# williamleif/GraphSAGE

Hardware: NVIDIA H100
Metric: seed_nodes_per_sec (higher is better)
Workload: dtype f32

## Files before the change

### graphsage_b200/_lib.py

```python
import ctypes
import os

import torch

_HERE = os.path.dirname(os.path.abspath(__file__))
LIB_PATH = os.path.join(_HERE, "csrc", "libgraphsage_b200.so")

ABI_VERSION = 2
GS_F32, GS_BF16, GS_F64, GS_I8ROW = 0, 1, 2, 3
ACT_NONE, ACT_RELU = 0, 1
COMBINE_ADD, COMBINE_CONCAT = 0, 1
MATH_FP32_SIMT, MATH_TF32X3, MATH_TF32, MATH_BF16 = 0, 1, 2, 3
CSR_MEAN, CSR_MEAN_SELF, CSR_MAX, CSR_SUM = 0, 1, 2, 3
MAX_SEGMENTS = 4

c_i32, c_i64, c_u64, c_vp = ctypes.c_int32, ctypes.c_int64, ctypes.c_uint64, ctypes.c_void_p


class Segment(ctypes.Structure):
    _fields_ = [("self_ids", c_vp), ("neigh_ids", c_vp), ("self_row0", c_i64), ("neigh_row0", c_i64),
                ("n", c_i64), ("k", c_i32), ("_pad", c_i32), ("out_row0", c_i64)]


MAX_SHARDS = 16


class ShardedTable(ctypes.Structure):
    _fields_ = [("base", c_vp * MAX_SHARDS), ("row_start", c_i64 * (MAX_SHARDS + 1)), ("n_shards", c_i32),
                ("my_shard", c_i32), ("n_global_rows", c_i64), ("zero_row", c_i64), ("remap", c_vp)]


class GemmPart(ctypes.Structure):
    _fields_ = [("A", c_vp), ("lda", c_i64), ("K", c_i32), ("B", c_vp), ("ldb", c_i64), ("N", c_i32)]


class RowRange(ctypes.Structure):
    _fields_ = [("ids", c_vp), ("row0", c_i64), ("n", c_i64)]


class GemmRowIds(ctypes.Structure):
    _fields_ = [("n_table_rows", c_i64), ("n_ranges", c_i32), ("_pad", c_i32), ("ranges", RowRange * MAX_SEGMENTS)]


MAX_EMBED_LISTS = 8
# ... 1 lines not shown
UNIQUE_DRAW_BUDGET = 1 << 20
WALK_MAX_WALKS = 1 << 20
WALK_MAX_LEN = 33
WALK_PQ_MIN, WALK_PQ_MAX = 1e-4, 1e4
MAX_BLOCK_LAYERS = 8
MAX_FANOUT = 256


class EmbedGradList(ctypes.Structure):
    _fields_ = [("ids", c_vp), ("grad", c_vp), ("ldg", c_i64), ("n", c_i64), ("group", c_i32), ("scale", ctypes.c_float)]


class DropoutSite(ctypes.Structure):
    _fields_ = [("seed", c_u64), ("call", ctypes.c_uint32), ("rate", ctypes.c_float), ("call_dev", c_vp)]


_SIGNATURES = {
    "gs_version": (c_i32, []),
    "gs_last_error_string": (ctypes.c_char_p, []),
    "gs_set_tuning": (c_i32, [ctypes.c_char_p, c_i32]),
    "gs_sample_padded": (c_i32, [c_vp, c_i64, c_i32, c_vp, c_i64, c_i32, c_vp, c_u64, c_u64, c_vp, c_vp, c_vp]),
    "gs_sample_padded_khop": (c_i32, [c_vp, c_i64, c_i32, c_vp, c_i64, ctypes.POINTER(c_i32), c_i32, c_u64, c_u64, c_vp,
                                      ctypes.POINTER(c_vp), c_vp]),
    "gs_build_padded_adj": (c_i32, [c_vp, c_vp, c_i64, c_i32, c_vp, c_u64, c_u64, c_vp, c_vp, c_vp]),
    "gs_sample_unigram": (c_i32, [c_vp, c_i64, c_i32, c_u64, c_u64, c_vp, c_vp, c_vp]),
    "gs_sample_unigram_unique": (c_i32, [c_vp, c_i64, c_i32, c_u64, c_u64, c_vp, c_vp, c_vp, c_vp]),
    "gs_sample_csr": (c_i32, [c_vp, c_vp, c_i64, c_vp, c_i64, c_i32, c_i32, c_u64, c_u64, c_vp, c_i32, c_vp, c_vp]),
    "gs_perm_prefix_host": (c_i32, [c_u64, c_u64, c_i32, c_i32, ctypes.POINTER(c_i32)]),
    "gs_gather_rows": (c_i32, [c_vp, c_i32, c_i64, c_i32, c_i64, c_vp, c_i64, c_vp, c_i64, c_vp]),
    "gs_gather_mean": (c_i32, [c_vp, c_i32, c_i64, c_i32, c_i64, ctypes.POINTER(Segment), c_i32, c_i32, c_vp, c_vp,
                               c_i64, c_vp]),
    "gs_gather_mean_sharded": (c_i32, [ctypes.POINTER(ShardedTable), c_i32, c_i32, c_i64, ctypes.POINTER(Segment), c_i32,
                                       c_i32, c_i32, c_vp, c_vp, c_vp, c_i64, c_vp]),
    "gs_halo_begin": (c_i32, [c_vp, c_i64, c_vp, c_vp]),
    "gs_halo_claim": (c_i32, [ctypes.POINTER(ShardedTable), c_vp, c_i64, c_vp, c_vp, c_vp, c_i64, c_vp]),
    "gs_halo_fetch": (c_i32, [ctypes.POINTER(ShardedTable), c_i32, c_i64, c_vp, c_vp, c_i64, c_vp, c_i64, c_vp]),
    "gs_halo_translate": (c_i32, [ctypes.POINTER(ShardedTable), c_vp, c_i64, c_vp, c_vp, c_vp]),
    "gs_translate_ids": (c_i32, [ctypes.POINTER(ShardedTable), c_vp, c_i64, c_vp, c_vp]),
    "gs_gather_rows_sharded": (c_i32, [ctypes.POINTER(ShardedTable), c_i32, c_i32, c_i64, c_vp, c_i64, c_vp, c_i64, c_vp]),
    "gs_shard_alloc": (c_i32, [c_i64, ctypes.POINTER(c_vp)]),
    "gs_shard_free": (c_i32, [c_vp]),
    "gs_ipc_export": (c_i32, [c_vp, ctypes.c_char_p]),
    "gs_ipc_import": (c_i32, [ctypes.c_char_p, ctypes.POINTER(c_vp)]),
    "gs_ipc_close": (c_i32, [c_vp]),
    "gs_host_register": (c_i32, [c_vp, c_i64, ctypes.POINTER(c_vp)]),
    "gs_host_unregister": (c_i32, [c_vp]),
# ... 157 lines not shown
```

### graphsage_b200/csrc/gather.cu

```cuda
#include "common.cuh"

namespace gs {

struct SegTable {
  gs_segment s[GS_MAX_SEGMENTS];
  int32_t n_segments;
  int64_t total_rows;
};

__device__ __forceinline__ int find_segment(const SegTable& t, int64_t r, int64_t& local) {
  int si = 0;
  int64_t base = 0, end = 0;
#pragma unroll
  for (int q = 0; q < GS_MAX_SEGMENTS - 1; ++q) {
    if (q < t.n_segments - 1) {
      end += t.s[q].n;
      if (r >= end) {
        base = end;
        si = q + 1;
      }
    }
  }
  local = r - base;
  return si;
// ... 223 lines not shown
  if (threadIdx.x == 0) {
    mbar_init(&bar[0], 1);
    mbar_init(&bar[1], 1);
    fence_mbar_init();
  }
  if constexpr (kDrop) {
    if (threadIdx.x < 2 * GS_MAX_SEGMENTS) {
      const int s = threadIdx.x % GS_MAX_SEGMENTS;
      drop_off[threadIdx.x] = drop_call_offset(threadIdx.x < GS_MAX_SEGMENTS ? drop.neigh[s] : drop.self[s]);
    }
  }
  __syncthreads();
  const int ncol4 = (int)(out_pitch >> 2);
  const int row_f4 = row_bytes >> 4;
  const size_t buf_bytes = (size_t)kGroupRows * row_bytes;
  const int self_rows = (include_self || out_self) ? 1 : 0;

  int64_t r_issue = blockIdx.x;
  int g_issue = 0;
  auto issue = [&](int buf) -> bool {
    if (r_issue >= tab.total_rows) return false;
    int64_t i;
    const gs_segment& sg = tab.s[find_segment(tab, r_issue, i)];
    const int k = sg.k;
    const int rows_total = k + self_rows;
    const int first = g_issue * kGroupRows;
    const int cnt = min(kGroupRows, rows_total - first);
    if (threadIdx.x < 32) {
      if (threadIdx.x == 0) mbar_expect_tx(&bar[buf], (uint32_t)(cnt * row_bytes));
      __syncwarp();
      for (int j = threadIdx.x; j < cnt; j += 32) {
        const int jj = first + j;
        int64_t id;
        if (jj < k) id = sg.neigh_ids ? (int64_t)sg.neigh_ids[i * k + jj] : sg.neigh_row0 + i * k + jj;
        else id = sg.self_ids ? (int64_t)sg.self_ids[i] : sg.self_row0 + i;
        bulk_g2s(smem + buf * buf_bytes + (size_t)j * row_bytes, rows_of.row(id), (uint32_t)row_bytes, &bar[buf]);
      }
    }
    if (first + cnt >= rows_total) { r_issue += gridDim.x; g_issue = 0; } else { ++g_issue; }
    return true;
  };

  uint32_t phase[2] = {0u, 0u};
  int buf = 0;
  bool have = issue(0);
  int64_t r = blockIdx.x;
  int g = 0;
  float4 acc[2];
  acc[0] = acc[1] = make_float4(0.f, 0.f, 0.f, 0.f);
  while (have) {
    const bool have_next = issue(buf ^ 1);
    int64_t i;
    const int si = find_segment(tab, r, i);
    const gs_segment& sg = tab.s[si];
    const int k = sg.k;
    const int rows_total = k + self_rows;
    const int first = g * kGroupRows;
    const int cnt = min(kGroupRows, rows_total - first);
    const bool last = first + cnt >= rows_total;
    mbar_wait(&bar[buf], phase[buf]);
    phase[buf] ^= 1u;
    const float4* rows = reinterpret_cast<const float4*>(smem + buf * buf_bytes);
    const int nn = last ? cnt - self_rows : cnt;
    DropSite nsite{};
    if constexpr (kDrop) nsite = with_call_offset(drop.neigh[si], drop_off[si]);
#pragma unroll
    for (int q = 0; q < 2; ++q) {
      const int c = threadIdx.x + q * blockDim.x;
      if (c < ncol4 && c * 4 < F) {
        float4 a = acc[q];
        for (int j = 0; j < nn; ++j) {
          float4 v = rows[j * row_f4 + c];
          if constexpr (kDrop) v = drop4(nsite, i * k + first + j, (uint32_t)c, v);
          a.x += v.x; a.y += v.y; a.z += v.z; a.w += v.w;
        }
        acc[q] = a;
      }
// ... 1108 lines not shown
```

### graphsage_b200/csrc/sampler.cu

```cuda
#include "common.cuh"

namespace gs {

constexpr int kMaxDegSmem = 1024;

__global__ void __launch_bounds__(256) sample_padded_kernel(const int32_t* __restrict__ adj, int64_t n_rows,
                                                            int32_t max_deg, const int32_t* __restrict__ ids,
                                                            int64_t n, int32_t k,
                                                            const int32_t* __restrict__ col_perm, uint64_t seed,
                                                            uint64_t counter, const uint64_t* __restrict__ counter_dev,
                                                            int32_t* __restrict__ out) {
  __shared__ int16_t perm[kMaxDegSmem];
  __shared__ int32_t pi[kMaxDegSmem];
  if (col_perm != nullptr) {
    for (int j = threadIdx.x; j < k; j += blockDim.x) pi[j] = col_perm[j];
  } else {
    for (int j = threadIdx.x; j < max_deg; j += blockDim.x) perm[j] = (int16_t)j;
    __syncthreads();
    if (threadIdx.x == 0) {
      uint64_t ctr = counter + (counter_dev ? *counter_dev : 0ull);
      u32x4 r{0, 0, 0, 0};
      for (int i = 0; i < k; ++i) {
        if ((i & 3) == 0) {
          u32x4 c{(uint32_t)ctr, (uint32_t)(ctr >> 32), 0u, kStreamPadded + (uint32_t)(i >> 2)};
// ... 5 lines not shown
        perm[j] = t;
        pi[i] = perm[i];
      }
    }
  }
  __syncthreads();
  const int64_t total = n * (int64_t)k;
  for (int64_t e = (int64_t)blockIdx.x * blockDim.x + threadIdx.x; e < total; e += (int64_t)gridDim.x * blockDim.x) {
    int64_t i = e / k;
    int j = (int)(e - i * k);
    int64_t id = ids[i];
    if (id < 0 || id >= n_rows) id = n_rows - 1;
    out[e] = adj[id * max_deg + pi[j]];
  }
}

struct KhopParams {
  int32_t* out[GS_MAX_HOPS];
  int32_t fanout[GS_MAX_HOPS];
  int64_t count[GS_MAX_HOPS];
  int32_t n_hops;
};

__global__ void __launch_bounds__(512) sample_padded_khop_kernel(const int32_t* __restrict__ adj, int64_t n_rows,
                                                                 int32_t max_deg, const int32_t* __restrict__ seeds,
                                                                 const __grid_constant__ KhopParams kp, uint64_t seed,
                                                                 uint64_t counter,
                                                                 const uint64_t* __restrict__ counter_dev) {
  __shared__ int16_t perm[GS_MAX_HOPS][kMaxDegSmem];
  __shared__ int32_t pi[GS_MAX_HOPS][64];
  const int warp = threadIdx.x >> 5, lane = threadIdx.x & 31;
  if (warp < kp.n_hops) {
    for (int j = lane; j < max_deg; j += 32) perm[warp][j] = (int16_t)j;
    __syncwarp();
    const uint64_t ctr = counter + (counter_dev ? *counter_dev : 0ull) + (uint64_t)warp;
    const int k = kp.fanout[warp];
    for (int blk = lane; blk * 4 < k; blk += 32) {
      u32x4 c{(uint32_t)ctr, (uint32_t)(ctr >> 32), 0u, kStreamPadded + (uint32_t)blk};
      u32x4 r = philox4x32_10(c, (uint32_t)seed, (uint32_t)(seed >> 32));
      pi[warp][blk * 4 + 0] = (int32_t)r.x;
      if (blk * 4 + 1 < 64) pi[warp][blk * 4 + 1] = (int32_t)r.y;
      if (blk * 4 + 2 < 64) pi[warp][blk * 4 + 2] = (int32_t)r.z;
      if (blk * 4 + 3 < 64) pi[warp][blk * 4 + 3] = (int32_t)r.w;
    }
    __syncwarp();
    if (lane == 0) {
      for (int i = 0; i < k; ++i) {
        int j = i + (int)mulhi32((uint32_t)pi[warp][i], (uint32_t)(max_deg - i));
        int16_t t = perm[warp][i];
        perm[warp][i] = perm[warp][j];
        perm[warp][j] = t;
        pi[warp][i] = perm[warp][i];
      }
    }
  }
  __syncthreads();
  int64_t total = 0;
  for (int t = 0; t < kp.n_hops; ++t) total += kp.count[t];
  for (int64_t e = (int64_t)blockIdx.x * blockDim.x + threadIdx.x; e < total; e += (int64_t)gridDim.x * blockDim.x) {
    int hop = 0;
    int64_t local = e;
    while (local >= kp.count[hop]) { local -= kp.count[hop]; ++hop; }
    int64_t sup = 1;
    for (int t = 0; t <= hop; ++t) sup *= kp.fanout[t];
    int64_t id = seeds[local / sup];
    int64_t rem = local % sup;
    for (int t = 0; t <= hop; ++t) {
      sup /= kp.fanout[t];
      const int j = (int)(rem / sup);
      rem -= (int64_t)j * sup;
      if (id < 0 || id >= n_rows) id = n_rows - 1;
      id = adj[id * max_deg + pi[t][j]];
    }
    kp.out[hop][local] = (int32_t)id;
  }
}

__global__ void __launch_bounds__(256) sample_csr_kernel(const int64_t* __restrict__ indptr,
                                                         const int32_t* __restrict__ indices, int64_t n_nodes,
                                                         const int32_t* __restrict__ ids, int64_t n, int32_t k,
                                                         int32_t replace_if_short, uint64_t seed, uint64_t counter,
                                                         const uint64_t* __restrict__ counter_dev, int32_t pad_id,
// ... 117 lines not shown
      for (int j = lane; j < max_deg; j += 32) {
        const uint32_t r = philox_draw(seed, counter, (uint32_t)u, kStreamBuild, j);
        row[j] = indices[start + (int64_t)mulhi32(r, (uint32_t)deg)];
      }
    } else {
      for (int j = 0; j < max_deg; ++j) {
        const int64_t m = deg - max_deg + j;
        const uint32_t r = philox_draw(seed, counter, (uint32_t)u, kStreamBuild, j);
        const int32_t t = (int32_t)mulhi32(r, (uint32_t)(m + 1));
        bool dup = false;
        for (int q = lane; q < j; q += 32) dup |= (sel[w][q] == t);
        dup = __any_sync(0xffffffffu, dup);
        if (lane == 0) sel[w][j] = dup ? (int32_t)m : t;
        __syncwarp();
      }
      for (int j = lane; j < max_deg; j += 32) row[j] = indices[start + sel[w][j]];
      __syncwarp();
    }
  }
}

}

extern "C" {

int32_t gs_sample_padded(const int32_t* adj, int64_t n_rows, int32_t max_deg, const int32_t* ids, int64_t n, int32_t k,
                         const int32_t* col_perm, uint64_t seed, uint64_t counter, const uint64_t* counter_dev,
                         int32_t* out, void* stream) {
  GS_REQUIRE(n >= 0 && k >= 0, "gs_sample_padded: negative size (n=%lld, k=%d)", (long long)n, k);
  if (n == 0 || k == 0) return GS_OK;
  GS_REQUIRE(adj && ids && out, "gs_sample_padded: NULL pointer");
  GS_REQUIRE(n_rows > 0 && max_deg > 0 && max_deg <= gs::kMaxDegSmem, "gs_sample_padded: need 0 < max_deg <= %d (got %d)",
             gs::kMaxDegSmem, max_deg);
  GS_REQUIRE(k <= max_deg, "gs_sample_padded: num_samples %d > max_degree %d", k, max_deg);
  int64_t total = n * (int64_t)k;
  int64_t blocks = (total + 255) / 256;
  int64_t cap = (int64_t)gs::sm_count() * 8;
  if (blocks > cap) blocks = cap;
  gs::sample_padded_kernel<<<(unsigned)blocks, 256, 0, (cudaStream_t)stream>>>(adj, n_rows, max_deg, ids, n, k, col_perm,
                                                                               seed, counter, counter_dev, out);
  return gs::launch_check("sample_padded_kernel");
}

int32_t gs_sample_padded_khop(const int32_t* adj, int64_t n_rows, int32_t max_deg, const int32_t* seeds, int64_t n_seeds,
                              const int32_t* fanout_host, int32_t n_hops, uint64_t seed, uint64_t counter,
                              const uint64_t* counter_dev, int32_t* const* out_host, void* stream) {
  GS_REQUIRE(n_hops >= 1 && n_hops <= GS_MAX_HOPS, "gs_sample_padded_khop: n_hops=%d (max %d)", n_hops, GS_MAX_HOPS);
  GS_REQUIRE(fanout_host && out_host, "gs_sample_padded_khop: NULL host array");
  GS_REQUIRE(n_seeds >= 0, "gs_sample_padded_khop: n_seeds < 0");
  if (n_seeds == 0) return GS_OK;
  GS_REQUIRE(adj && seeds, "gs_sample_padded_khop: NULL pointer");
  GS_REQUIRE(n_rows > 0 && max_deg > 0 && max_deg <= gs::kMaxDegSmem, "gs_sample_padded_khop: need 0 < max_deg <= %d",
             gs::kMaxDegSmem);
  gs::KhopParams kp;
  memset(&kp, 0, sizeof(kp));
  kp.n_hops = n_hops;
  int64_t cnt = n_seeds, total = 0;
  for (int t = 0; t < n_hops; ++t) {
    GS_REQUIRE(fanout_host[t] >= 1 && fanout_host[t] <= max_deg && fanout_host[t] <= 64,
               "gs_sample_padded_khop: fanout[%d]=%d (need 1..min(64, max_degree))", t, fanout_host[t]);
    GS_REQUIRE(out_host[t] != nullptr, "gs_sample_padded_khop: out[%d] is NULL", t);
    cnt *= fanout_host[t];
    kp.fanout[t] = fanout_host[t];
    kp.count[t] = cnt;
    kp.out[t] = out_host[t];
    total += cnt;
  }
  int64_t blocks = (total + 511) / 512;
  int64_t cap = (int64_t)gs::sm_count() * 2;
  if (blocks > cap) blocks = cap;
  gs::sample_padded_khop_kernel<<<(unsigned)blocks, 512, 0, (cudaStream_t)stream>>>(adj, n_rows, max_deg, seeds, kp, seed,
                                                                                    counter, counter_dev);
  return gs::launch_check("sample_padded_khop_kernel");
}

int32_t gs_build_padded_adj(const int64_t* indptr, const int32_t* indices, int64_t n_nodes, int32_t max_deg,
                            const uint8_t* skip, uint64_t seed, uint64_t counter, int32_t* adj, float* deg, void* stream) {
  GS_REQUIRE(indptr && indices && adj && n_nodes >= 0, "gs_build_padded_adj: NULL pointer / bad size");
  GS_REQUIRE(max_deg >= 1 && max_deg <= gs::kMaxDegSmem, "gs_build_padded_adj: need 1 <= max_deg <= %d", gs::kMaxDegSmem);
  int64_t blocks = (n_nodes + 1 + 7) / 8;
  int64_t cap = (int64_t)gs::sm_count() * 4;
  if (blocks > cap) blocks = cap;
  gs::build_padded_adj_kernel<<<(unsigned)blocks, 256, 0, (cudaStream_t)stream>>>(indptr, indices, n_nodes, max_deg, skip,
                                                                                   seed, counter, adj, deg);
  return gs::launch_check("build_padded_adj_kernel");
}

int32_t gs_sample_unigram(const double* cdf, int64_t n, int32_t num_sampled, uint64_t seed, uint64_t counter,
                          const uint64_t* counter_dev, int32_t* out, void* stream) {
  GS_REQUIRE(num_sampled >= 0 && n >= 1, "gs_sample_unigram: bad sizes");
  if (num_sampled == 0) return GS_OK;
  GS_REQUIRE(cdf && out, "gs_sample_unigram: NULL pointer");
  gs::sample_unigram_kernel<<<(num_sampled + 127) / 128, 128, 0, (cudaStream_t)stream>>>(cdf, n, num_sampled, seed, counter,
                                                                                       counter_dev, out);
  return gs::launch_check("sample_unigram_kernel");
// ... 36 lines not shown
```

### graphsage_b200/models.py

```python
from collections import namedtuple

import numpy as np
import torch

from . import ops
from .aggregators import (GCNAggregator, MaxPoolingAggregator, MeanAggregator, MeanPoolingAggregator, SeqAggregator,
                          TwoMaxLayerPoolingAggregator, refuse_seq_table)
from .host_features import HostFeatures, refuse_host_table, stage_layer0, step_rows
from .int8_features import Int8Features, refuse_int8_table
from .layers import identity, relu

SAGEInfo = namedtuple("SAGEInfo",
                      ["layer_name",
                       "neigh_sampler",
                       "num_samples",
                       "output_dim"])

_AGGREGATORS = {"mean": MeanAggregator, "maxpool": MaxPoolingAggregator, "gcn": GCNAggregator,
                "meanpool": MeanPoolingAggregator, "seq": SeqAggregator,
                "twomaxpool": TwoMaxLayerPoolingAggregator}
_SIZED_AGGREGATORS = (MaxPoolingAggregator, SeqAggregator)


def layer_segments(samples, counts, num_samples, layer):
    L = len(num_samples)
    hops = L - layer
    row0 = [sum(counts[:h]) for h in range(hops + 1)]
    segs = []
    for hop in range(hops):
        k = num_samples[L - hop - 1]
        if layer == 0:
            segs.append(ops.Seg(counts[hop], k, self_ids=samples[hop], neigh_ids=samples[hop + 1], out_row0=row0[hop]))
        else:
            segs.append(ops.Seg(counts[hop], k, self_row0=row0[hop], neigh_row0=row0[hop + 1], out_row0=row0[hop]))
    return segs


class SampleAndAggregate(object):

    def __init__(self, placeholders, features, adj, degrees, layer_infos, concat=True, aggregator_type="mean",
                 model_size="small", identity_dim=0, device="cuda", **kwargs):
        allowed_kwargs = {"name", "logging", "model_size"}
        for kwarg in kwargs.keys():
            assert kwarg in allowed_kwargs, "Invalid keyword argument: " + kwarg
        if aggregator_type not in _AGGREGATORS:
            raise ValueError("Unknown aggregator: %r" % (aggregator_type,))
        self.aggregator_cls = _AGGREGATORS[aggregator_type]
        if features is None and not identity_dim > 0:
            raise ValueError("Must have a positive value for identity feature dimension if no input features given.")
        self.placeholders = placeholders if placeholders is not None else {}
        self.inputs1 = self.placeholders.get("batch1")
        self.inputs2 = self.placeholders.get("batch2")
        self.model_size = model_size
        self.adj_info = adj
        self.identity_dim, self.embeds = int(identity_dim), None
# ... 48 lines not shown
            raise ValueError("features has %d rows, the adjacency table %d: both must be [N+1, .] (dummy row last)"
                             % (features.shape[0], n_rows))
        F_ = 0 if features is None else int(features.shape[1])
        table = torch.zeros((n_rows, ops.pad_cols(d + F_)), dtype=torch.float32, device=device)
        table[:, :d] = glorot([n_rows, d], name="node_embeddings", device=device)
        if F_:
            table[:, d:d + F_] = features.to(device=device)
        self.features = table[:, :d + F_]
        self.embeds = table[:, :d]

    def _finish_init(self, placeholders, adj, degrees, layer_infos, concat, model_size, identity_dim, device):
        if self.aggregator_cls is SeqAggregator:
            refuse_seq_table(self.features)
        self.degrees = degrees
        self.concat = concat
        self.dims = [self.features.shape[1] + identity_dim]
        self.dims.extend([layer_infos[i].output_dim for i in range(len(layer_infos))])
        self.batch_size = self.placeholders.get("batch_size")
        self.layer_infos = layer_infos
        self.device = torch.device(device)
        self.aggregators = None

    def sample(self, inputs, layer_infos, batch_size=None):
        if batch_size is None:
            batch_size = self.batch_size if self.batch_size is not None else inputs.numel()
        samples = [inputs.reshape(-1)]
        support_size = 1
        support_sizes = [support_size]
        L = len(layer_infos)
        fan = [layer_infos[L - k - 1].num_samples for k in range(L)]
        s0 = layer_infos[0].neigh_sampler
        if (L <= 4 and hasattr(s0, "sample_khop") and all(i.neigh_sampler is s0 for i in layer_infos)
                and max(fan) <= 64 and samples[0].numel() == batch_size):
            for k, ids in enumerate(s0.sample_khop(samples[0], fan)):
                support_size *= fan[k]
                samples.append(ids)
                support_sizes.append(support_size)
            return samples, support_sizes
        for k in range(len(layer_infos)):
            t = len(layer_infos) - k - 1
            support_size *= layer_infos[t].num_samples
            sampler = layer_infos[t].neigh_sampler
            node = sampler((samples[k], layer_infos[t].num_samples))
            samples.append(node.reshape(support_size * batch_size))
            support_sizes.append(support_size)
        return samples, support_sizes

    def aggregate(self, samples, input_features, dims, num_samples, support_sizes, batch_size=None,
                  aggregators=None, name=None, concat=False, model_size="small", _final=None):
        if batch_size is None:
            batch_size = self.batch_size if self.batch_size is not None else samples[0].numel()
        feats = input_features[0] if isinstance(input_features, (list, tuple)) else input_features
        L = len(num_samples)
        new_agg = aggregators is None
        if new_agg:
            aggregators = []
            for layer in range(L):
                dim_mult = 2 if concat and (layer != 0) else 1
                act = identity if layer == L - 1 else relu
                kw = dict(act=act, dropout=self.placeholders.get("dropout", 0.), name=name, concat=concat,
                          device=self.device)
                if issubclass(self.aggregator_cls, _SIZED_AGGREGATORS):
                    kw["model_size"] = model_size
                aggregators.append(self.aggregator_cls(dim_mult * dims[layer], dims[layer + 1], **kw))
        if any(getattr(a, "dropout", 0.) and not isinstance(a, SeqAggregator) for a in aggregators):
            return self._aggregate_materialised(samples, feats, dims, num_samples, support_sizes, batch_size,
                                                aggregators, concat), aggregators
        counts = [batch_size * support_sizes[h] for h in range(L + 1)]
        src, samples, persistent = stage_layer0(feats, samples)
        for layer in range(L):
            src = aggregators[layer].aggregate_rows(src, layer_segments(samples, counts, num_samples, layer),
                                                    final=_final if layer == L - 1 else None,
                                                    src_persistent=(layer == 0 and persistent))
        return src[:counts[0]], aggregators

    def _aggregate_materialised(self, samples, feats, dims, num_samples, support_sizes, batch_size, aggregators,
                                concat):
        feats, samples, _ = stage_layer0(feats, samples)
        hidden = [ops.gather_rows(feats, s) for s in samples]
        L = len(num_samples)
        for layer in range(L):
            nxt = []
            for hop in range(L - layer):
                d = hidden[hop + 1].shape[1]
                neigh = hidden[hop + 1].reshape(batch_size * support_sizes[hop], num_samples[L - hop - 1], d)
                nxt.append(aggregators[layer]((hidden[hop], neigh)))
            hidden = nxt
        return hidden[0]

    def graphed(self, batch_size, normalize=True, probe=None):
        return GraphedForward(self, batch_size, normalize, probe)

    def pipelined(self, batch_size, normalize=True, depth=2):
        return PipelinedForward(self, batch_size, normalize, depth)
# ... 15 lines not shown
        from .full_neighbor_training import full_neighbor_embeddings
        return full_neighbor_embeddings(self, indptr, indices, node_ids, normalize)

    def full_neighbor_minibatch_embeddings(self, indptr, indices, node_ids, normalize=True):
        from .full_neighbor_training import full_neighbor_embeddings
        return full_neighbor_embeddings(self, indptr, indices, node_ids, normalize, minibatch=True)

    def sampled_minibatch_embeddings(self, indptr, indices, node_ids, normalize=True):
        from .full_neighbor_training import full_neighbor_embeddings
        return full_neighbor_embeddings(self, indptr, indices, node_ids, normalize, minibatch=True, sampled=True)

    def _csr_input(self, t, dtype, name):
        if not torch.is_tensor(t):
            arr = np.asarray(t)
            if arr.dtype != {torch.int64: np.int64, torch.int32: np.int32}[dtype]:
                raise TypeError("%s must be %s (got %s)" % (name, dtype, arr.dtype))
            return torch.as_tensor(arr, device=self.device)
        if t.dtype != dtype:
            raise TypeError("%s must be %s (got %s)" % (name, dtype, t.dtype))
        if t.device != self.device and not (t.is_cuda and self.device.type == "cuda" and self.device.index is None):
            raise ValueError("%s is on %s, the model on %s" % (name, t.device, self.device))
        return t.contiguous()

    def forward(self, batch, normalize=True):
        batch = batch.to(device=self.device, dtype=torch.int32).reshape(-1)
        n = batch.numel()
        samples, support = self.sample(batch, self.layer_infos, batch_size=n)
        num_samples = [info.num_samples for info in self.layer_infos]
        final = {"l2_normalize": bool(normalize), "bump": getattr(self, "_graph_bump", None)}
        out, self.aggregators = self.aggregate(samples, [self.features], self.dims, num_samples, support,
                                               batch_size=n, aggregators=self.aggregators, concat=self.concat,
                                               model_size=self.model_size, _final=final)
        if normalize and not final.get("normalized"):
            out = ops.l2_normalize_rows_(out.contiguous())
        if final["bump"] is not None and not final.get("bumped"):
            ops.check(ops.lib().gs_bump_counter(final["bump"][0].data_ptr(), int(final["bump"][1]), ops.stream_ptr()))
            ops._launched(1)
        return out


class GraphedForward(object):

    def __init__(self, model, batch_size, normalize=True, probe=None, first_step=0, step_stride=1):
        self.model, self.batch_size, self.normalize = model, int(batch_size), normalize
        dev = model.device
        self.ids = torch.zeros(self.batch_size, dtype=torch.int32, device=dev)
        self.first_step, self.step_stride = int(first_step), int(step_stride)
        self.counter = torch.full((1,), len(model.layer_infos) * self.first_step, dtype=torch.int64, device=dev)
        samplers = []
        for info in model.layer_infos:
            if all(info.neigh_sampler is not s for s in samplers):
                samplers.append(info.neigh_sampler)
        if len(samplers) != 1:
            raise NotImplementedError("GraphedForward needs all layer_infos to share one neigh_sampler object")
        self.samplers = samplers
# ... 159 lines not shown
```

### graphsage_b200/neigh_samplers.py

```python
import torch

from . import ops
from .layers import Layer


class UniformNeighborSampler(Layer):

    def __init__(self, adj_info, seed=123, **kwargs):
        super(UniformNeighborSampler, self).__init__(**kwargs)
        self.set_adj(adj_info)
        self.seed = int(seed)
        self.counter = 0
        self.counter_dev = None

    def set_adj(self, adj_info):
        if adj_info.dtype != torch.int32 or adj_info.dim() != 2:
            raise TypeError("adj_info must be an int32 [N+1, max_degree] tensor")
        ops.require_cuda(adj_info)
        self.adj_info = adj_info.contiguous()

    def _call(self, inputs):
        ids, num_samples = inputs
        out = ops.sample_padded(self.adj_info, ids, int(num_samples), self.seed, self.counter,
                                counter_dev=self.counter_dev)
        self.counter += 1
        return out

    def sample_khop(self, ids, fanouts):
        outs = ops.sample_padded_khop(self.adj_info, ids, [int(k) for k in fanouts], self.seed, self.counter,
                                      counter_dev=self.counter_dev)
        self.counter += len(fanouts)
        return outs


class CSRNeighborSampler(Layer):

    def __init__(self, indptr, indices, seed=123, replace_if_short=True, pad_id=None, **kwargs):
        super(CSRNeighborSampler, self).__init__(**kwargs)
        ops.require_cuda(indptr, indices)
        self.indptr, self.indices = indptr.contiguous(), indices.contiguous()
        self.seed = int(seed)
        self.counter = 0
        self.counter_dev = None
        self.replace_if_short = replace_if_short
        self.pad_id = int(indptr.numel() - 1) if pad_id is None else int(pad_id)

    def _call(self, inputs):
        ids, num_samples = inputs
        out = ops.sample_csr(self.indptr, self.indices, ids, int(num_samples), self.seed, self.counter,
                             self.replace_if_short, self.pad_id, counter_dev=self.counter_dev)
        self.counter += 1
        return out
```

### graphsage_b200/ops.py

```python
import collections
import math

import torch

from . import _lib
from ._lib import (ACT_NONE, ACT_RELU, COMBINE_ADD, COMBINE_CONCAT, MATH_FP32_SIMT, MATH_TF32X3, MATH_TF32,
                   MATH_BF16, GemmPart, GemmRowIds, RowRange, Segment, check, lib, ptr, require_cuda, stream_ptr)

_U64 = 2**64 - 1

PROBE = None
LAUNCHES = 0
STAGE_HOOK = None

CACHE_EPOCH = [0]
REPACK_ALWAYS = [False]


def _probe(name):
    if STAGE_HOOK is not None:
        STAGE_HOOK(name, "pre")
    if PROBE is None:
        return _PostHook(name) if STAGE_HOOK is not None else None
    e0, e1 = torch.cuda.Event(enable_timing=True), torch.cuda.Event(enable_timing=True)
# ... 21 lines not shown
def pad_cols(f):
    return (int(f) + 7) // 8 * 8


def _i32(t, name):
    if t.dtype != torch.int32:
        raise TypeError("%s must be int32 (got %s)" % (name, t.dtype))
    return t.contiguous()


def sample_padded(adj, ids, k, seed, counter, col_perm=None, counter_dev=None, out=None):
    require_cuda(adj, ids, col_perm, counter_dev)
    adj, ids = _i32(adj, "adj"), _i32(ids.reshape(-1), "ids")
    n = ids.numel()
    if out is None:
        out = torch.empty((n, k), dtype=torch.int32, device=adj.device)
    ev = _probe("sample_padded")
    check(lib().gs_sample_padded(ptr(adj), adj.shape[0], adj.shape[1], ptr(ids), n, k, ptr(col_perm), seed & _U64,
                                 counter & _U64, ptr(counter_dev), ptr(out), stream_ptr()))
    _launched(1 if n * k else 0, ev)
    return out


def sample_padded_khop(adj, seeds, fanouts, seed, counter, counter_dev=None):
    require_cuda(adj, seeds, counter_dev)
    adj, seeds = _i32(adj, "adj"), _i32(seeds.reshape(-1), "seeds")
    n = seeds.numel()
    outs, cnt = [], n
    for k in fanouts:
        cnt *= int(k)
        outs.append(torch.empty((cnt,), dtype=torch.int32, device=adj.device))
    fan = (_lib.c_i32 * len(fanouts))(*[int(k) for k in fanouts])
    optr = (_lib.c_vp * len(fanouts))(*[ptr(o) for o in outs])
    ev = _probe("sample_padded_khop")
    check(lib().gs_sample_padded_khop(ptr(adj), adj.shape[0], adj.shape[1], ptr(seeds), n, fan, len(fanouts),
                                      seed & _U64, counter & _U64, ptr(counter_dev), optr, stream_ptr()))
    _launched(1 if n else 0, ev)
    return outs


def build_padded_adj(indptr, indices, max_degree, seed=123, counter=0, skip=None):
    require_cuda(indptr, indices, skip)
    if indptr.dtype != torch.int64:
        raise TypeError("indptr must be int64")
    indices = _i32(indices, "indices")
    n = indptr.numel() - 1
    adj = torch.empty((n + 1, max_degree), dtype=torch.int32, device=indptr.device)
    deg = torch.empty((n,), dtype=torch.float32, device=indptr.device)
    sk = None if skip is None else skip.to(torch.uint8).contiguous()
    check(lib().gs_build_padded_adj(ptr(indptr), ptr(indices), n, max_degree, ptr(sk), seed & _U64, counter & _U64,
                                    ptr(adj), ptr(deg), stream_ptr()))
    _launched(1)
    return adj, deg


def sample_unigram(cdf, num_sampled, seed, counter, counter_dev=None):
    require_cuda(cdf, counter_dev)
    if cdf.dtype != torch.float64:
        raise TypeError("cdf must be float64")
    out = torch.empty((num_sampled,), dtype=torch.int32, device=cdf.device)
    check(lib().gs_sample_unigram(ptr(cdf), cdf.numel(), num_sampled, seed & _U64, counter & _U64, ptr(counter_dev),
# ... 186 lines not shown
    if out.dtype != torch.float32 or out.stride(1) != 1 or out.shape[0] < n:
        raise ValueError("out must be a row-major float32 matrix with >= n rows")
    src, code, n_rows, pitch = _table(feats)
    check(lib().gs_gather_rows_f32(src, code, n_rows, F, pitch, ptr(ids), int(row0), n, ptr(out), out.stride(0), stream_ptr()))
    _launched(1 if n else 0)
    return out


def cast_rows_bf16(x, out=None):
    require_cuda(x, out)
    if x.dtype != torch.float32 or x.dim() != 2 or x.stride(1) != 1:
        raise ValueError("x must be a row-major float32 matrix")
    n, F = x.shape
    if out is None:
        out = torch.empty((n, pad_cols(F)), dtype=torch.bfloat16, device=x.device)[:, :F]
    if out.dtype != torch.bfloat16 or out.stride(1) != 1 or out.shape[0] < n or out.stride(0) < F:
        raise ValueError("out must be a row-major bfloat16 matrix with >= n rows")
    check(lib().gs_cast_rows_bf16(ptr(x), n, F, x.stride(0), ptr(out), out.stride(0), stream_ptr()))
    _launched(1 if n else 0)
    return out


class Seg(object):
    __slots__ = ("n", "k", "self_ids", "neigh_ids", "self_row0", "neigh_row0", "out_row0")

    def __init__(self, n, k, self_ids=None, neigh_ids=None, self_row0=0, neigh_row0=0, out_row0=0):
        self.n, self.k = int(n), int(k)
        self.self_ids = None if self_ids is None else _i32(self_ids.reshape(-1), "self_ids")
        self.neigh_ids = None if neigh_ids is None else _i32(neigh_ids.reshape(-1), "neigh_ids")
        self.self_row0, self.neigh_row0, self.out_row0 = int(self_row0), int(neigh_row0), int(out_row0)
        if self.self_ids is not None and self.self_ids.numel() < self.n:
            raise ValueError("self_ids shorter than n")
        if self.neigh_ids is not None and self.neigh_ids.numel() < self.n * self.k:
            raise ValueError("neigh_ids shorter than n*k")

    def c_struct(self):
        require_cuda(self.self_ids, self.neigh_ids)
        return Segment(ptr(self.self_ids), ptr(self.neigh_ids), self.self_row0, self.neigh_row0, self.n, self.k, 0,
                       self.out_row0)


def make_segment(n, k, self_ids=None, neigh_ids=None, self_row0=0, neigh_row0=0, out_row0=0):
    return Seg(n, k, self_ids, neigh_ids, self_row0, neigh_row0, out_row0)



def _check_out(t, rows, out_pitch, name):
    if t is None:
        return
    require_cuda(t)
    if t.dtype != torch.float32 or t.dim() != 2 or t.stride(1) != 1 or t.stride(0) != out_pitch or t.shape[0] < rows:
        raise ValueError("%s must be a float32 [>= %d, .] CUDA matrix with row stride out_pitch = %d" % (name, rows, out_pitch))


def gather_mean(src, segments, include_self=False, want_self=True, out_pitch=None, out_mean=None, out_self=None):
    if hasattr(src, "c_table"):
        return _gather_mean_sharded(src, segments, include_self, want_self, out_pitch, out_mean, out_self)
    if not isinstance(src, I8Rows):
        require_cuda(src)
        if src.dtype not in (torch.float32, torch.bfloat16) or src.dim() != 2 or src.stride(1) != 1:
            raise ValueError("src must be a row-major float32 (or bfloat16) 2-D tensor")
    F = src.shape[1]
# ... 921 lines not shown
```

### include/graphsage_b200.h

```cpp
#ifndef GRAPHSAGE_B200_H_
#define GRAPHSAGE_B200_H_

#include <stdint.h>

#ifdef __cplusplus
extern "C" {
#endif

#define GS_ABI_VERSION 2

typedef enum {
  GS_OK = 0,
  GS_ERR_INVALID_ARG = -1,
  GS_ERR_CUDA = -2,
  GS_ERR_UNSUPPORTED = -3
} gs_status;

typedef enum { GS_F32 = 0, GS_BF16 = 1, GS_F64 = 2, GS_I8ROW = 3 } gs_dtype;

int64_t gs_i8row_pitch(int32_t F);
int32_t gs_quantize_rows_i8(const float* x, int64_t n, int32_t F, int64_t ldx, void* out, int64_t out_pitch_bytes,
                            void* stream);
typedef enum { GS_ACT_NONE = 0, GS_ACT_RELU = 1 } gs_act;
typedef enum {
// ... 2 lines not shown
} gs_combine;
typedef enum {
  GS_MATH_FP32_SIMT = 0,
  GS_MATH_TF32X3 = 1,
  GS_MATH_TF32 = 2,
  GS_MATH_BF16 = 3
} gs_math;

int32_t gs_version(void);
const char* gs_last_error_string(void);
int32_t gs_set_tuning(const char* key, int32_t value);

int32_t gs_sample_padded(const int32_t* adj, int64_t n_rows, int32_t max_deg,
                         const int32_t* ids, int64_t n, int32_t k,
                         const int32_t* col_perm, uint64_t seed, uint64_t counter,
                         const uint64_t* counter_dev, int32_t* out, void* stream);

#define GS_MAX_HOPS 4
int32_t gs_sample_padded_khop(const int32_t* adj, int64_t n_rows, int32_t max_deg,
                              const int32_t* seeds, int64_t n_seeds, const int32_t* fanout_host,
                              int32_t n_hops, uint64_t seed, uint64_t counter,
                              const uint64_t* counter_dev, int32_t* const* out_host, void* stream);

int32_t gs_sample_csr(const int64_t* indptr, const int32_t* indices, int64_t n_nodes,
                      const int32_t* ids, int64_t n, int32_t k, int32_t replace_if_short,
                      uint64_t seed, uint64_t counter, const uint64_t* counter_dev,
                      int32_t pad_id, int32_t* out, void* stream);

int32_t gs_sample_unigram(const double* cdf, int64_t n, int32_t num_sampled, uint64_t seed, uint64_t counter,
                          const uint64_t* counter_dev, int32_t* out, void* stream);

#define GS_MAX_UNIQUE_SAMPLED 1024
#define GS_UNIQUE_DRAW_BUDGET (1 << 20)
int32_t gs_sample_unigram_unique(const double* cdf, int64_t n, int32_t num_sampled, uint64_t seed, uint64_t counter,
                                 const uint64_t* counter_dev, int32_t* out, int32_t* status, void* stream);

int32_t gs_build_padded_adj(const int64_t* indptr, const int32_t* indices, int64_t n_nodes, int32_t max_deg,
                            const uint8_t* skip, uint64_t seed, uint64_t counter, int32_t* adj, float* deg,
                            void* stream);

int32_t gs_perm_prefix_host(uint64_t seed, uint64_t counter, int32_t max_deg, int32_t k,
                            int32_t* out_host);

int32_t gs_gather_rows(const void* feats, int32_t dtype, int64_t n_rows, int32_t F,
                       int64_t pitch, const int32_t* ids, int64_t n, void* out,
                       int64_t out_pitch, void* stream);

#define GS_MAX_SEGMENTS 4
typedef struct {
  const int32_t* self_ids;
  const int32_t* neigh_ids;
  int64_t self_row0;
  int64_t neigh_row0;
  int64_t n;
  int32_t k;
  int32_t _pad;
  int64_t out_row0;
} gs_segment;

int32_t gs_gather_mean(const void* src, int32_t dtype, int64_t n_src_rows, int32_t F, int64_t pitch,
                       const gs_segment* segments_host, int32_t n_segments, int32_t include_self,
                       void* out_self, void* out_mean, int64_t out_pitch, void* stream);

#define GS_MAX_SHARDS 16
typedef struct {
  const void* base[GS_MAX_SHARDS];
  int64_t row_start[GS_MAX_SHARDS + 1];
  int32_t n_shards;
  int32_t my_shard;
  int64_t n_global_rows;
  int64_t zero_row;
  const int32_t* remap;
} gs_sharded_table;

int32_t gs_gather_mean_sharded(const gs_sharded_table* table_host, int32_t dtype, int32_t F, int64_t pitch,
                               const gs_segment* segments_host, int32_t n_segments, int32_t include_self,
                               int32_t ids_are_locators, const void* staging, void* out_self, void* out_mean,
                               int64_t out_pitch, void* stream);
int32_t gs_halo_begin(int32_t* claim, int64_t n_global_rows, int32_t* count, void* stream);
int32_t gs_halo_claim(const gs_sharded_table* table_host, const int32_t* ids, int64_t n, int32_t* claim, int32_t* count,
// ... 272 lines not shown
```

Before: 3.482 million.

## Bucket-sort hop-1 nodes by id range to localize layer-0 gather

Adds an ordered k-hop sampling variant in which one extra block computes a counting-sort permutation of hop-1 nodes, bucketed by the high bits of their node ids. The layer-0 gather-mean kernel then walks hop-1 rows in this permuted order, so blocks running at the same time fetch feature rows from nearby address ranges. The aim is better L2 locality when gathering neighbour features. The cost is a serial ranking pass on a single block, an extra indirection load per row, and a new ABI field in the segment struct.

```diff
diff --git a/graphsage_b200/_lib.py b/graphsage_b200/_lib.py
--- a/graphsage_b200/_lib.py
+++ b/graphsage_b200/_lib.py
@@ -19,7 +19,7 @@
 
 class Segment(ctypes.Structure):
     _fields_ = [("self_ids", c_vp), ("neigh_ids", c_vp), ("self_row0", c_i64), ("neigh_row0", c_i64),
-                ("n", c_i64), ("k", c_i32), ("_pad", c_i32), ("out_row0", c_i64)]
+                ("n", c_i64), ("k", c_i32), ("_pad", c_i32), ("out_row0", c_i64), ("order", c_vp)]
 
 
 MAX_SHARDS = 16
@@ -67,6 +67,9 @@
     "gs_sample_padded": (c_i32, [c_vp, c_i64, c_i32, c_vp, c_i64, c_i32, c_vp, c_u64, c_u64, c_vp, c_vp, c_vp]),
     "gs_sample_padded_khop": (c_i32, [c_vp, c_i64, c_i32, c_vp, c_i64, ctypes.POINTER(c_i32), c_i32, c_u64, c_u64, c_vp,
                                       ctypes.POINTER(c_vp), c_vp]),
+    "gs_order_shift": (c_i32, [c_i64]),
+    "gs_sample_padded_khop_ordered": (c_i32, [c_vp, c_i64, c_i32, c_vp, c_i64, ctypes.POINTER(c_i32), c_i32, c_u64, c_u64,
+                                              c_vp, ctypes.POINTER(c_vp), c_vp, c_vp]),
     "gs_build_padded_adj": (c_i32, [c_vp, c_vp, c_i64, c_i32, c_vp, c_u64, c_u64, c_vp, c_vp, c_vp]),
     "gs_sample_unigram": (c_i32, [c_vp, c_i64, c_i32, c_u64, c_u64, c_vp, c_vp, c_vp]),
     "gs_sample_unigram_unique": (c_i32, [c_vp, c_i64, c_i32, c_u64, c_u64, c_vp, c_vp, c_vp, c_vp]),
diff --git a/graphsage_b200/csrc/gather.cu b/graphsage_b200/csrc/gather.cu
--- a/graphsage_b200/csrc/gather.cu
+++ b/graphsage_b200/csrc/gather.cu
@@ -269,6 +269,7 @@
     if (r_issue >= tab.total_rows) return false;
     int64_t i;
     const gs_segment& sg = tab.s[find_segment(tab, r_issue, i)];
+    if (sg.order) i = sg.order[i];
     const int k = sg.k;
     const int rows_total = k + self_rows;
     const int first = g_issue * kGroupRows;
@@ -300,6 +301,7 @@
     int64_t i;
     const int si = find_segment(tab, r, i);
     const gs_segment& sg = tab.s[si];
+    if (sg.order) i = sg.order[i];
     const int k = sg.k;
     const int rows_total = k + self_rows;
     const int first = g * kGroupRows;
diff --git a/graphsage_b200/csrc/sampler.cu b/graphsage_b200/csrc/sampler.cu
--- a/graphsage_b200/csrc/sampler.cu
+++ b/graphsage_b200/csrc/sampler.cu
@@ -51,13 +51,108 @@
   int32_t n_hops;
 };
 
+constexpr int kRankWarps = 16;
+constexpr int kRankIter = 16;
+static_assert(GS_ORDER_BUCKETS < 256, "same_bucket_lanes compares 8 bits (the buckets and the past-the-chunk value)");
+
+__device__ __forceinline__ int32_t hop1_bucket(const int32_t* __restrict__ adj, int64_t n_rows, int32_t max_deg,
+                                               const int32_t* __restrict__ seeds, const int32_t* pi0, int32_t f0, int32_t e,
+                                               int32_t shift) {
+  int64_t id = seeds[e / f0];
+  if (id < 0 || id >= n_rows) id = n_rows - 1;
+  id = adj[id * max_deg + pi0[e % f0]];
+  if (id < 0 || id >= n_rows) id = n_rows - 1;
+  return (int32_t)(id >> shift);
+}
+
+__device__ __forceinline__ unsigned same_bucket_lanes(int32_t b) {
+  unsigned m = 0xffffffffu;
+#pragma unroll
+  for (int bit = 0; bit < 8; ++bit) {
+    const bool one = (b >> bit) & 1;
+    const unsigned bal = __ballot_sync(0xffffffffu, one);
+    m &= one ? bal : ~bal;
+  }
+  return m;
+}
+
+__device__ __forceinline__ void rank_hop1(const int32_t* __restrict__ adj, int64_t n_rows, int32_t max_deg,
+                                          const int32_t* __restrict__ seeds, const int32_t* pi0, int32_t f0, int32_t n1,
+                                          int32_t shift, int32_t* wcnt, int32_t* tot, int32_t* __restrict__ order) {
+  constexpr int B = GS_ORDER_BUCKETS;
+  const int warp = threadIdx.x >> 5, lane = threadIdx.x & 31;
+  const unsigned below = (1u << lane) - 1u;
+  for (int i = threadIdx.x; i < kRankWarps * B; i += blockDim.x) wcnt[i] = 0;
+  __syncthreads();
+  const int32_t chunk = (n1 + kRankWarps - 1) / kRankWarps;
+  const int32_t lo = min(n1, warp * chunk), hi = min(n1, lo + chunk);
+  const bool one_round = hi - lo <= 32 * kRankIter;
+  int32_t* mine = wcnt + warp * B;
+  int32_t b[kRankIter];
+  for (int pass = 0; pass < 2; ++pass) {
+    for (int32_t r0 = lo; r0 < hi; r0 += 32 * kRankIter) {
+      if (pass == 0 || !one_round) {
+#pragma unroll
+        for (int it = 0; it < kRankIter; ++it) {
+          const int32_t e = r0 + it * 32 + lane;
+          b[it] = e < hi ? hop1_bucket(adj, n_rows, max_deg, seeds, pi0, f0, e, shift) : B;
+        }
+      }
+#pragma unroll
+      for (int it = 0; it < kRankIter; ++it) {
+        if (r0 + it * 32 >= hi) break;
+        const unsigned same = same_bucket_lanes(b[it]);
+        if (pass == 1 && b[it] < B) order[mine[b[it]] + __popc(same & below)] = r0 + it * 32 + lane;
+        __syncwarp();
+        if (b[it] < B && (same & below) == 0u) mine[b[it]] += __popc(same);
+        __syncwarp();
+      }
+    }
+    __syncthreads();
+    if (pass == 0) {
+      if (threadIdx.x < B) {
+        int32_t s = 0;
+        for (int w = 0; w < kRankWarps; ++w) s += wcnt[w * B + threadIdx.x];
+        tot[threadIdx.x] = s;
+      }
+      __syncthreads();
+      if (warp == 0) {
+        int32_t v[B / 32], s = 0;
+#pragma unroll
+        for (int q = 0; q < B / 32; ++q) { v[q] = s; s += tot[lane * (B / 32) + q]; }
+        int32_t incl = s;
+#pragma unroll
+        for (int d = 1; d < 32; d <<= 1) {
+          const int32_t t = __shfl_up_sync(0xffffffffu, incl, d);
+          if (lane >= d) incl += t;
+        }
+#pragma unroll
+        for (int q = 0; q < B / 32; ++q) tot[lane * (B / 32) + q] = incl - s + v[q];
+      }
+      __syncthreads();
+      if (threadIdx.x < B) {
+        int32_t run = tot[threadIdx.x];
+        for (int w = 0; w < kRankWarps; ++w) {
+          const int32_t c = wcnt[w * B + threadIdx.x];
+          wcnt[w * B + threadIdx.x] = run;
+          run += c;
+        }
+      }
+      __syncthreads();
+    }
+  }
+}
+
 __global__ void __launch_bounds__(512) sample_padded_khop_kernel(const int32_t* __restrict__ adj, int64_t n_rows,
                                                                  int32_t max_deg, const int32_t* __restrict__ seeds,
                                                                  const __grid_constant__ KhopParams kp, uint64_t seed,
                                                                  uint64_t counter,
-                                                                 const uint64_t* __restrict__ counter_dev) {
-  __shared__ int16_t perm[GS_MAX_HOPS][kMaxDegSmem];
+                                                                 const uint64_t* __restrict__ counter_dev,
+                                                                 int32_t* __restrict__ order, int32_t order_shift) {
+  __shared__ __align__(16) int16_t perm[GS_MAX_HOPS][kMaxDegSmem];
   __shared__ int32_t pi[GS_MAX_HOPS][64];
+  __shared__ int32_t rank_tot[GS_ORDER_BUCKETS];
+  static_assert(sizeof(perm) >= kRankWarps * GS_ORDER_BUCKETS * sizeof(int32_t), "rank_hop1's counts live in perm");
   const int warp = threadIdx.x >> 5, lane = threadIdx.x & 31;
   if (warp < kp.n_hops) {
     for (int j = lane; j < max_deg; j += 32) perm[warp][j] = (int16_t)j;
@@ -84,9 +179,16 @@
     }
   }
   __syncthreads();
+  const int rank_blocks = order != nullptr ? 1 : 0;
+  if (rank_blocks && blockIdx.x == 0) {
+    rank_hop1(adj, n_rows, max_deg, seeds, pi[0], kp.fanout[0], (int32_t)kp.count[0], order_shift,
+              reinterpret_cast<int32_t*>(&perm[0][0]), rank_tot, order);
+    return;
+  }
   int64_t total = 0;
   for (int t = 0; t < kp.n_hops; ++t) total += kp.count[t];
-  for (int64_t e = (int64_t)blockIdx.x * blockDim.x + threadIdx.x; e < total; e += (int64_t)gridDim.x * blockDim.x) {
+  const int64_t stride = (int64_t)(gridDim.x - rank_blocks) * blockDim.x;
+  for (int64_t e = (int64_t)(blockIdx.x - rank_blocks) * blockDim.x + threadIdx.x; e < total; e += stride) {
     int hop = 0;
     int64_t local = e;
     while (local >= kp.count[hop]) { local -= kp.count[hop]; ++hop; }
@@ -250,6 +352,32 @@
 
 }
 
+static int32_t khop_params(const char* who, const int32_t* adj, int64_t n_rows, int32_t max_deg, const int32_t* seeds,
+                           int64_t n_seeds, const int32_t* fanout_host, int32_t n_hops, int32_t* const* out_host,
+                           gs::KhopParams& kp, int64_t& total) {
+  total = 0;
+  GS_REQUIRE(n_hops >= 1 && n_hops <= GS_MAX_HOPS, "%s: n_hops=%d (max %d)", who, n_hops, GS_MAX_HOPS);
+  GS_REQUIRE(fanout_host && out_host, "%s: NULL host array", who);
+  GS_REQUIRE(n_seeds >= 0, "%s: n_seeds < 0", who);
+  if (n_seeds == 0) return GS_OK;
+  GS_REQUIRE(adj && seeds, "%s: NULL pointer", who);
+  GS_REQUIRE(n_rows > 0 && max_deg > 0 && max_deg <= gs::kMaxDegSmem, "%s: need 0 < max_deg <= %d", who, gs::kMaxDegSmem);
+  memset(&kp, 0, sizeof(kp));
+  kp.n_hops = n_hops;
+  int64_t cnt = n_seeds;
+  for (int t = 0; t < n_hops; ++t) {
+    GS_REQUIRE(fanout_host[t] >= 1 && fanout_host[t] <= max_deg && fanout_host[t] <= 64,
+               "%s: fanout[%d]=%d (need 1..min(64, max_degree))", who, t, fanout_host[t]);
+    GS_REQUIRE(out_host[t] != nullptr, "%s: out[%d] is NULL", who, t);
+    cnt *= fanout_host[t];
+    kp.fanout[t] = fanout_host[t];
+    kp.count[t] = cnt;
+    kp.out[t] = out_host[t];
+    total += cnt;
+  }
+  return GS_OK;
+}
+
 extern "C" {
 
 int32_t gs_sample_padded(const int32_t* adj, int64_t n_rows, int32_t max_deg, const int32_t* ids, int64_t n, int32_t k,
@@ -270,35 +398,45 @@
   return gs::launch_check("sample_padded_kernel");
 }
 
+int32_t gs_order_shift(int64_t n_rows) {
+  int32_t s = 12;
+  while (s < 62 && ((n_rows - 1) >> s) >= GS_ORDER_BUCKETS) ++s;
+  return s;
+}
+
 int32_t gs_sample_padded_khop(const int32_t* adj, int64_t n_rows, int32_t max_deg, const int32_t* seeds, int64_t n_seeds,
                               const int32_t* fanout_host, int32_t n_hops, uint64_t seed, uint64_t counter,
                               const uint64_t* counter_dev, int32_t* const* out_host, void* stream) {
-  GS_REQUIRE(n_hops >= 1 && n_hops <= GS_MAX_HOPS, "gs_sample_padded_khop: n_hops=%d (max %d)", n_hops, GS_MAX_HOPS);
-  GS_REQUIRE(fanout_host && out_host, "gs_sample_padded_khop: NULL host array");
-  GS_REQUIRE(n_seeds >= 0, "gs_sample_padded_khop: n_seeds < 0");
-  if (n_seeds == 0) return GS_OK;
-  GS_REQUIRE(adj && seeds, "gs_sample_padded_khop: NULL pointer");
-  GS_REQUIRE(n_rows > 0 && max_deg > 0 && max_deg <= gs::kMaxDegSmem, "gs_sample_padded_khop: need 0 < max_deg <= %d",
-             gs::kMaxDegSmem);
   gs::KhopParams kp;
-  memset(&kp, 0, sizeof(kp));
-  kp.n_hops = n_hops;
-  int64_t cnt = n_seeds, total = 0;
-  for (int t = 0; t < n_hops; ++t) {
-    GS_REQUIRE(fanout_host[t] >= 1 && fanout_host[t] <= max_deg && fanout_host[t] <= 64,
-               "gs_sample_padded_khop: fanout[%d]=%d (need 1..min(64, max_degree))", t, fanout_host[t]);
-    GS_REQUIRE(out_host[t] != nullptr, "gs_sample_padded_khop: out[%d] is NULL", t);
-    cnt *= fanout_host[t];
-    kp.fanout[t] = fanout_host[t];
-    kp.count[t] = cnt;
-    kp.out[t] = out_host[t];
-    total += cnt;
-  }
+  int64_t total = 0;
+  const int32_t rc = khop_params("gs_sample_padded_khop", adj, n_rows, max_deg, seeds, n_seeds, fanout_host, n_hops, out_host,
+                                 kp, total);
+  if (rc != GS_OK || total == 0) return rc;
   int64_t blocks = (total + 511) / 512;
   int64_t cap = (int64_t)gs::sm_count() * 2;
   if (blocks > cap) blocks = cap;
   gs::sample_padded_khop_kernel<<<(unsigned)blocks, 512, 0, (cudaStream_t)stream>>>(adj, n_rows, max_deg, seeds, kp, seed,
-                                                                                    counter, counter_dev);
+                                                                                    counter, counter_dev, nullptr, 0);
+  return gs::launch_check("sample_padded_khop_kernel");
+}
+
+int32_t gs_sample_padded_khop_ordered(const int32_t* adj, int64_t n_rows, int32_t max_deg, const int32_t* seeds,
+                                      int64_t n_seeds, const int32_t* fanout_host, int32_t n_hops, uint64_t seed,
+                                      uint64_t counter, const uint64_t* counter_dev, int32_t* const* out_host, int32_t* order,
+                                      void* stream) {
+  gs::KhopParams kp;
+  int64_t total = 0;
+  const int32_t rc = khop_params("gs_sample_padded_khop_ordered", adj, n_rows, max_deg, seeds, n_seeds, fanout_host, n_hops,
+                                 out_host, kp, total);
+  if (rc != GS_OK || total == 0) return rc;
+  GS_REQUIRE(order != nullptr, "gs_sample_padded_khop_ordered: order is NULL");
+  GS_REQUIRE(kp.count[0] < (int64_t)INT32_MAX - 32 * gs::kRankIter,
+             "gs_sample_padded_khop_ordered: %lld hop-1 ids (order is int32)", (long long)kp.count[0]);
+  int64_t blocks = (total + 511) / 512;
+  int64_t cap = (int64_t)gs::sm_count() * 2;
+  if (blocks > cap) blocks = cap;
+  gs::sample_padded_khop_kernel<<<(unsigned)(blocks + 1), 512, 0, (cudaStream_t)stream>>>(
+      adj, n_rows, max_deg, seeds, kp, seed, counter, counter_dev, order, gs_order_shift(n_rows));
   return gs::launch_check("sample_padded_khop_kernel");
 }
 
diff --git a/graphsage_b200/models.py b/graphsage_b200/models.py
--- a/graphsage_b200/models.py
+++ b/graphsage_b200/models.py
@@ -22,7 +22,7 @@
 _SIZED_AGGREGATORS = (MaxPoolingAggregator, SeqAggregator)
 
 
-def layer_segments(samples, counts, num_samples, layer):
+def layer_segments(samples, counts, num_samples, layer, hop1_order=None):
     L = len(num_samples)
     hops = L - layer
     row0 = [sum(counts[:h]) for h in range(hops + 1)]
@@ -30,7 +30,8 @@
     for hop in range(hops):
         k = num_samples[L - hop - 1]
         if layer == 0:
-            segs.append(ops.Seg(counts[hop], k, self_ids=samples[hop], neigh_ids=samples[hop + 1], out_row0=row0[hop]))
+            segs.append(ops.Seg(counts[hop], k, self_ids=samples[hop], neigh_ids=samples[hop + 1], out_row0=row0[hop],
+                                order=hop1_order if hop == 1 else None))
         else:
             segs.append(ops.Seg(counts[hop], k, self_row0=row0[hop], neigh_row0=row0[hop + 1], out_row0=row0[hop]))
     return segs
@@ -125,6 +126,9 @@
         self.aggregators = None
 
     def sample(self, inputs, layer_infos, batch_size=None):
+        return self._sample(inputs, layer_infos, batch_size)[:2]
+
+    def _sample(self, inputs, layer_infos, batch_size=None, hop1_order=False):
         if batch_size is None:
             batch_size = self.batch_size if self.batch_size is not None else inputs.numel()
         samples = [inputs.reshape(-1)]
@@ -135,11 +139,13 @@
         s0 = layer_infos[0].neigh_sampler
         if (L <= 4 and hasattr(s0, "sample_khop") and all(i.neigh_sampler is s0 for i in layer_infos)
                 and max(fan) <= 64 and samples[0].numel() == batch_size):
-            for k, ids in enumerate(s0.sample_khop(samples[0], fan)):
+            outs = s0.sample_khop(samples[0], fan, hop1_order=hop1_order)
+            outs, order = outs if hop1_order else (outs, None)
+            for k, ids in enumerate(outs):
                 support_size *= fan[k]
                 samples.append(ids)
                 support_sizes.append(support_size)
-            return samples, support_sizes
+            return samples, support_sizes, order
         for k in range(len(layer_infos)):
             t = len(layer_infos) - k - 1
             support_size *= layer_infos[t].num_samples
@@ -147,10 +153,10 @@
             node = sampler((samples[k], layer_infos[t].num_samples))
             samples.append(node.reshape(support_size * batch_size))
             support_sizes.append(support_size)
-        return samples, support_sizes
+        return samples, support_sizes, None
 
     def aggregate(self, samples, input_features, dims, num_samples, support_sizes, batch_size=None,
-                  aggregators=None, name=None, concat=False, model_size="small", _final=None):
+                  aggregators=None, name=None, concat=False, model_size="small", _final=None, _hop1_order=None):
         if batch_size is None:
             batch_size = self.batch_size if self.batch_size is not None else samples[0].numel()
         feats = input_features[0] if isinstance(input_features, (list, tuple)) else input_features
@@ -172,7 +178,8 @@
         counts = [batch_size * support_sizes[h] for h in range(L + 1)]
         src, samples, persistent = stage_layer0(feats, samples)
         for layer in range(L):
-            src = aggregators[layer].aggregate_rows(src, layer_segments(samples, counts, num_samples, layer),
+            segs = layer_segments(samples, counts, num_samples, layer, _hop1_order if layer == 0 else None)
+            src = aggregators[layer].aggregate_rows(src, segs,
                                                     final=_final if layer == L - 1 else None,
                                                     src_persistent=(layer == 0 and persistent))
         return src[:counts[0]], aggregators
@@ -234,15 +241,20 @@
             raise ValueError("%s is on %s, the model on %s" % (name, t.device, self.device))
         return t.contiguous()
 
+    def _orders_hop1(self):
+        f = self.features
+        return (self.aggregator_cls is MeanAggregator and len(self.layer_infos) >= 2 and torch.is_tensor(f)
+                and f.is_cuda and f.dtype == torch.float32 and not self.placeholders.get("dropout", 0.))
+
     def forward(self, batch, normalize=True):
         batch = batch.to(device=self.device, dtype=torch.int32).reshape(-1)
         n = batch.numel()
-        samples, support = self.sample(batch, self.layer_infos, batch_size=n)
+        samples, support, order = self._sample(batch, self.layer_infos, batch_size=n, hop1_order=self._orders_hop1())
         num_samples = [info.num_samples for info in self.layer_infos]
         final = {"l2_normalize": bool(normalize), "bump": getattr(self, "_graph_bump", None)}
         out, self.aggregators = self.aggregate(samples, [self.features], self.dims, num_samples, support,
                                                batch_size=n, aggregators=self.aggregators, concat=self.concat,
-                                               model_size=self.model_size, _final=final)
+                                               model_size=self.model_size, _final=final, _hop1_order=order)
         if normalize and not final.get("normalized"):
             out = ops.l2_normalize_rows_(out.contiguous())
         if final["bump"] is not None and not final.get("bumped"):
diff --git a/graphsage_b200/neigh_samplers.py b/graphsage_b200/neigh_samplers.py
--- a/graphsage_b200/neigh_samplers.py
+++ b/graphsage_b200/neigh_samplers.py
@@ -26,9 +26,9 @@
         self.counter += 1
         return out
 
-    def sample_khop(self, ids, fanouts):
+    def sample_khop(self, ids, fanouts, hop1_order=False):
         outs = ops.sample_padded_khop(self.adj_info, ids, [int(k) for k in fanouts], self.seed, self.counter,
-                                      counter_dev=self.counter_dev)
+                                      counter_dev=self.counter_dev, hop1_order=hop1_order)
         self.counter += len(fanouts)
         return outs
 
diff --git a/graphsage_b200/ops.py b/graphsage_b200/ops.py
--- a/graphsage_b200/ops.py
+++ b/graphsage_b200/ops.py
@@ -67,7 +67,7 @@
     return out
 
 
-def sample_padded_khop(adj, seeds, fanouts, seed, counter, counter_dev=None):
+def sample_padded_khop(adj, seeds, fanouts, seed, counter, counter_dev=None, hop1_order=False):
     require_cuda(adj, seeds, counter_dev)
     adj, seeds = _i32(adj, "adj"), _i32(seeds.reshape(-1), "seeds")
     n = seeds.numel()
@@ -78,10 +78,16 @@
     fan = (_lib.c_i32 * len(fanouts))(*[int(k) for k in fanouts])
     optr = (_lib.c_vp * len(fanouts))(*[ptr(o) for o in outs])
     ev = _probe("sample_padded_khop")
-    check(lib().gs_sample_padded_khop(ptr(adj), adj.shape[0], adj.shape[1], ptr(seeds), n, fan, len(fanouts),
-                                      seed & _U64, counter & _U64, ptr(counter_dev), optr, stream_ptr()))
+    if hop1_order:
+        order = torch.empty_like(outs[0])
+        check(lib().gs_sample_padded_khop_ordered(ptr(adj), adj.shape[0], adj.shape[1], ptr(seeds), n, fan, len(fanouts),
+                                                  seed & _U64, counter & _U64, ptr(counter_dev), optr, ptr(order),
+                                                  stream_ptr()))
+    else:
+        check(lib().gs_sample_padded_khop(ptr(adj), adj.shape[0], adj.shape[1], ptr(seeds), n, fan, len(fanouts),
+                                          seed & _U64, counter & _U64, ptr(counter_dev), optr, stream_ptr()))
     _launched(1 if n else 0, ev)
-    return outs
+    return (outs, order) if hop1_order else outs
 
 
 def build_padded_adj(indptr, indices, max_degree, seed=123, counter=0, skip=None):
@@ -314,22 +320,25 @@
 
 
 class Seg(object):
-    __slots__ = ("n", "k", "self_ids", "neigh_ids", "self_row0", "neigh_row0", "out_row0")
-
-    def __init__(self, n, k, self_ids=None, neigh_ids=None, self_row0=0, neigh_row0=0, out_row0=0):
+    __slots__ = ("n", "k", "self_ids", "neigh_ids", "self_row0", "neigh_row0", "out_row0", "order")
+
+    def __init__(self, n, k, self_ids=None, neigh_ids=None, self_row0=0, neigh_row0=0, out_row0=0, order=None):
         self.n, self.k = int(n), int(k)
         self.self_ids = None if self_ids is None else _i32(self_ids.reshape(-1), "self_ids")
         self.neigh_ids = None if neigh_ids is None else _i32(neigh_ids.reshape(-1), "neigh_ids")
+        self.order = None if order is None else _i32(order.reshape(-1), "order")
         self.self_row0, self.neigh_row0, self.out_row0 = int(self_row0), int(neigh_row0), int(out_row0)
         if self.self_ids is not None and self.self_ids.numel() < self.n:
             raise ValueError("self_ids shorter than n")
         if self.neigh_ids is not None and self.neigh_ids.numel() < self.n * self.k:
             raise ValueError("neigh_ids shorter than n*k")
+        if self.order is not None and self.order.numel() != self.n:
+            raise ValueError("order must hold n entries")
 
     def c_struct(self):
-        require_cuda(self.self_ids, self.neigh_ids)
+        require_cuda(self.self_ids, self.neigh_ids, self.order)
         return Segment(ptr(self.self_ids), ptr(self.neigh_ids), self.self_row0, self.neigh_row0, self.n, self.k, 0,
-                       self.out_row0)
+                       self.out_row0, ptr(self.order))
 
 
 def make_segment(n, k, self_ids=None, neigh_ids=None, self_row0=0, neigh_row0=0, out_row0=0):
diff --git a/include/graphsage_b200.h b/include/graphsage_b200.h
--- a/include/graphsage_b200.h
+++ b/include/graphsage_b200.h
@@ -48,6 +48,14 @@
                               int32_t n_hops, uint64_t seed, uint64_t counter,
                               const uint64_t* counter_dev, int32_t* const* out_host, void* stream);
 
+#define GS_ORDER_BUCKETS 128
+int32_t gs_order_shift(int64_t n_rows);
+int32_t gs_sample_padded_khop_ordered(const int32_t* adj, int64_t n_rows, int32_t max_deg,
+                                      const int32_t* seeds, int64_t n_seeds, const int32_t* fanout_host,
+                                      int32_t n_hops, uint64_t seed, uint64_t counter,
+                                      const uint64_t* counter_dev, int32_t* const* out_host, int32_t* order,
+                                      void* stream);
+
 int32_t gs_sample_csr(const int64_t* indptr, const int32_t* indices, int64_t n_nodes,
                       const int32_t* ids, int64_t n, int32_t k, int32_t replace_if_short,
                       uint64_t seed, uint64_t counter, const uint64_t* counter_dev,
@@ -82,6 +90,7 @@
   int32_t k;
   int32_t _pad;
   int64_t out_row0;
+  const int32_t* order;
 } gs_segment;
 
 int32_t gs_gather_mean(const void* src, int32_t dtype, int64_t n_src_rows, int32_t F, int64_t pitch,
```

New measurement: 3.343 million (median of 6 runs). 4.0% lower.
